# MacPhobos/audio-ident

Hardware: AMD Instinct MI355X
Metric: audio-seconds fingerprinted/sec/GPU; landmark-hash bit-exact vs CPU ref (higher is better)
Workload: dtype f32; 1 GPU; BASELINE configs[1]: 256 x 10 s 44.1 kHz mono clips, fingerprint extraction per GPU; clips_per_gpu=256, n_fft=2048, hop=512, parallelism=clip-sharded x1 (no data-path collective)

## Files before the change

audio-ident_amd/csrc/aidfp_extract.h:

```cpp
#pragma once
#include "aidfp_buffers.h"
#include "aidfp_extract_plan.h"

namespace aid {

struct Extractor {
    DevBuf<float> pcm_stage, power;
    DevBuf<uint64_t> mask, hotw;
    DevBuf<uint32_t> clip_qmax;
    DevBuf<uint32_t> k2_cold;
    HostBuf<uint64_t> h_cold;
    uint64_t *h_cold_dev = nullptr;
    DevBuf<int64_t> chunk_counts, counts;
    DevBuf<uint64_t> records;
    DevBuf<ClipDesc> desc;
    HostBuf<ClipDesc> h_desc;
    size_t desc_n = 0;
    ClipDesc *desc_dev = nullptr;
    Event desc_ev, stage_ev;
    hipStream_t stage_stream = nullptr;
    K2Policy k2;
    int64_t k2_slots[2] = {1, 1};
    int64_t k1_slots = 1;
    int64_t plane_rows = 0;
    ExtractPlan plan;
    bool have_result = false;
};

}
```

audio-ident_amd/csrc/aidfp_launch.h:

```cpp
#pragma once
#include <hip/hip_runtime.h>
#include <stdint.h>

#include "aidfp_device.h"

namespace aid {
void launch_stft_power(const void *pcm, bool s16, const ClipDesc *clips, int n_clips, int64_t f0, int64_t total_frames,
                       int64_t total_strips, int64_t slots, int hop, const Tables *tab, float *out, bool logmag,
                       uint64_t *hot, float thr, bool keep_power, uint32_t *qmax, hipStream_t s);
int peak_pick_blocks_per_cu(int width);
void launch_peak_pick(int width, const float *power, const ClipDesc *clips, int n_clips, int64_t f0, int64_t total_strips,
                      int strip_len, float thr, const uint64_t *hot, uint64_t *mask, uint32_t *cold_cnt,
                      const uint32_t *clip_qmax, float rel, hipStream_t s);
void launch_landmarks(const uint64_t *mask, const ClipDesc *clips, int n_clips, int64_t total_chunks,
                      int64_t *chunk_counts, uint64_t *records, int64_t *clip_counts, bool write, uint32_t *k2_cold,
                      uint64_t *k2_cold_host, uint32_t k2_waves, uint32_t k2_strips, bool one_chunk_each,
                      hipStream_t s);
void launch_synth(float *out, const uint32_t *tracks, const int64_t *starts, int n_clips, int64_t n, int sr,
                  int noise_a, uint32_t salt, int fmax_hz, bool envelope, const int16_t *sin_tab, hipStream_t s);
void launch_resample(const void *src, bool s16, int64_t in_base, int64_t n, int channels, int up, int down, int hl,
                     int J, const float *taps, float *dst, int64_t m_first, int64_t count, hipStream_t s,
                     int n_streams = 1, int64_t src_stride = 0, int64_t dst_stride = 0, const void *hist = nullptr,
                     int64_t hist_n = 0, int64_t hist_stride = 0);
struct SpeedVarDev;
void launch_resample_speeds(const void *src, bool s16, int channels, const int64_t *clip_off, const SpeedVarDev *vars,
                            int n_speeds, const int64_t *blk_first, const int64_t *dst_off, int pair0, int n_pairs,
                            int64_t blocks, int64_t lds_floats, float *dst, hipStream_t s);
void launch_s16_to_f32(const int16_t *src, int64_t n, float *dst, hipStream_t s);
int dedup_chunks(int64_t n_cat);
void launch_dedup_scan(const uint32_t *cw, const int64_t *coff, const double *cdur, int64_t n_cat, const uint32_t *qw,
                       const int64_t *qoff, const double *qlo, const double *qhi, int nq, double *part_sim,
                       int64_t *part_idx, double *best_sim, int64_t *best_idx, hipStream_t s);
void launch_dedup_pairs(const uint32_t *aw, const int64_t *aoff, const uint32_t *bw, const int64_t *boff, int n,
                        double *sim, hipStream_t s);
void launch_index_count(const uint32_t *ph, const uint32_t *ptrack, int64_t n, const uint8_t *tomb, uint32_t n_tracks,
                        uint32_t *cnt, hipStream_t s);
void launch_index_scatter(const uint32_t *ph, const uint32_t *ptrack, const uint32_t *pt, int64_t n,
                          const uint8_t *tomb, uint32_t n_tracks, uint32_t *cursor, uint64_t *post, hipStream_t s);
void launch_scan(const uint32_t *in, uint32_t *out, int64_t n, uint32_t *tmp, hipStream_t s);
int match_lds_blocks_per_cu();
size_t radix_scratch_u32(int64_t n);
hipError_t launch_index_sort_build(const uint32_t *ph, const uint32_t *ptrack, const uint32_t *pt, int64_t n,
                                   const uint8_t *tomb, uint32_t n_tracks, uint32_t *keys0, uint32_t *keys1,
                                   uint64_t *vals0, uint64_t *vals1, uint32_t *scratch, uint32_t *E, uint32_t *offsets,
                                   unsigned long long *nz, uint64_t **vals_out, uint16_t *sig, int rank_mode,
                                   hipStream_t s);
void launch_make_sig(const uint64_t *post, int64_t n, uint16_t *sig, hipStream_t s);
// ... 48 lines not shown
```

audio-ident_amd/csrc/aidfp_layout.h:

```cpp
#pragma once
#include <stdint.h>

namespace aid {

constexpr int kN = 2048;
constexpr int kBins = 1024;
constexpr int kPeakDT = 7;
constexpr int kPeakDF = 15;
constexpr int kZoneDT = 63;
constexpr int kZoneDF = 127;
constexpr int kFan = 10;
constexpr int kMaskWords = kBins / 64;

constexpr int kStftWaves = 16;
constexpr int kStftStrip = 16;
constexpr int kK1MinFrames = 2;
constexpr int kStftLdsPerWave = 1092;

constexpr int kPeakStripMin = 16;
constexpr int kPeakStripMax = 65536;

inline int peak_strip_len(const int64_t *frames, int n, int64_t slots) {
    int64_t fmax = 0;
    for (int c = 0; c < n; ++c) fmax = frames[c] > fmax ? frames[c] : fmax;
    auto count = [&](int64_t L) {
        int64_t k = 0;
        for (int c = 0; c < n; ++c) k += (frames[c] + L - 1) / L;
        return k;
    };
    int64_t lo = kPeakStripMin, hi = fmax > lo ? fmax : lo;
    if (hi > kPeakStripMax) hi = kPeakStripMax;
    if (count(lo) <= slots) return (int)lo;
    while (lo < hi) {
        const int64_t mid = (lo + hi) / 2;
        if (count(mid) <= slots) hi = mid; else lo = mid + 1;
    }
    return (int)lo;
}

constexpr int hot_bit(int c) { return c < 32 ? c : 95 - c; }

__host__ __device__ constexpr uint32_t bucket_key(uint32_t h) {
    return (((h >> 22) & 0xFFu) << 18) | ((h >> 30) << 16) | (((h >> 12) & 0x7Fu) << 9) | (((h >> 19) & 0x7u) << 6) |
           (h & 0x3Fu);
}

__host__ __device__ constexpr uint16_t posting_sig(uint32_t track, uint32_t t) {
    return (uint16_t)(((track * 0x9E3779B1u) >> 16) + t);
}

constexpr int64_t kLdsMaxVotes = (int64_t)1 << 18;

constexpr int kHashChunk = 1024;
constexpr int kHashChunkPeakCap = 64 * ((kHashChunk + kZoneDT + 7) / 8);

inline int64_t num_frames(int64_t n, int hop) { return (hop <= 0 || n < kN) ? 0 : 1 + (n - kN) / hop; }
inline int64_t peak_capacity(int64_t F) { return 64 * ((F + 7) / 8); }
inline int64_t hash_capacity(int64_t F) { return kFan * peak_capacity(F); }

struct ClipDesc {
    int64_t pcm_off;
    int64_t frames;
    int64_t frame_base;
    int64_t strip_base;
    int64_t chunk_base;
    int64_t hash_base;
    int64_t hash_cap;
    int64_t stft_base;
};

}
```

audio-ident_amd/csrc/extract.cpp:

```cpp
#include <cstring>

#include "engine_internal.h"

int extract_locked(aid_engine *e, const void *pcm, PcmFmt fmt, const int64_t *offsets, int32_t n_clips, int32_t loc,
                   void *stream, const int64_t *ends) {
    if (ends && loc != AID_PCM_DEVICE) return fail(AID_ERR_INVALID, "extract: clip ends need device PCM");
    HIP_TRY(hipSetDevice(e->device));
    Extractor &x = e->ext;
    ExtractPlan &p = x.plan;
    hipStream_t s = pick_stream(e, stream);
    const bool keep_power = (e->cfg.flags & AID_FLAG_KEEP_POWER) != 0, rel = e->cfg.peak_rel > 0.0f;
    if (e->last_stream && e->last_stream != s) HIP_TRY(hipStreamSynchronize(e->last_stream));
    x.have_result = false;
    const uint64_t cw = x.h_cold.p ? *reinterpret_cast<volatile uint64_t *>(x.h_cold.p) : 0;
    const uint64_t sw = x.h_cold.p ? *reinterpret_cast<volatile uint64_t *>(x.h_cold.p + 1) : 0;
    const K2Choice k2 = x.k2.choose(cw, sw);
    plan_extract(p, offsets, ends, n_clips, loc, e->cfg.hop, x.plane_rows, keep_power,
                 x.k2_slots[k2.width == 2 ? 0 : 1], k2.slots_x, k2.width);
    int64_t plane = 1;
    for (const ClipGroup &g : p.groups) plane = std::max(plane, g.frames);
    HIP_TRY(x.desc.reserve((size_t)n_clips + 1));
    HIP_TRY(x.power.reserve((size_t)plane * kBins));
    HIP_TRY(x.mask.reserve((size_t)p.total_frames * kMaskWords));
    HIP_TRY(x.hotw.reserve((size_t)p.total_frames + 1));
    if (rel) {
        HIP_TRY(x.clip_qmax.reserve((size_t)n_clips + 1));
        if (n_clips > 0) HIP_TRY(hipMemsetAsync(x.clip_qmax.p, 0, sizeof(uint32_t) * (size_t)n_clips, s));
    }
    if (!x.h_cold.p) {
        HIP_TRY(x.k2_cold.reserve(128));
        HIP_TRY(hipMemsetAsync(x.k2_cold.p, 0, 128 * sizeof(uint32_t), s));
        HIP_TRY(x.h_cold.reserve(2, hipHostMallocMapped));
        x.h_cold.p[0] = x.h_cold.p[1] = 0;
        HIP_TRY(hipHostGetDevicePointer((void **)&x.h_cold_dev, x.h_cold.p, 0));
    }
    HIP_TRY(x.chunk_counts.reserve((size_t)p.chunks + 1));
    HIP_TRY(x.records.reserve((size_t)p.records + 1));
    HIP_TRY(x.counts.reserve((size_t)n_clips + 1));
    const void *dpcm = pcm;
    if (p.staged > 0) {
        if (x.stage_stream != s) HIP_TRY(x.stage_ev.wait());
        x.stage_ev.live = false;
        const size_t nbytes = (size_t)p.staged * pcm_size(fmt);
        HIP_TRY(x.pcm_stage.reserve((nbytes + sizeof(float) - 1) / sizeof(float)));
        HIP_TRY(hipMemcpyAsync(x.pcm_stage.p, pcm_at(pcm, fmt, offsets[0]), nbytes, hipMemcpyHostToDevice, s));
        dpcm = x.pcm_stage.p;
    }
    if (n_clips > 0 && (x.desc_dev != x.desc.p || desc_differ(p.desc.data(), (size_t)n_clips, x.h_desc.p, x.desc_n))) {
        x.desc_dev = nullptr;
        HIP_TRY(x.desc_ev.wait());
        HIP_TRY(x.h_desc.reserve((size_t)n_clips + 1));
        std::memcpy(x.h_desc.p, p.desc.data(), sizeof(ClipDesc) * n_clips);
        HIP_TRY(hipMemcpyAsync(x.desc.p, x.h_desc.p, sizeof(ClipDesc) * n_clips, hipMemcpyHostToDevice, s));
        HIP_TRY(x.desc_ev.record(s));
        x.desc_n = (size_t)n_clips;
        x.desc_dev = x.desc.p;
    }
    if (p.empty_clip || p.total_frames == 0)
        HIP_TRY(hipMemsetAsync(x.counts.p, 0, sizeof(int64_t) * ((size_t)n_clips + 1), s));
    if (p.total_frames > 0) {
        for (const ClipGroup &g : p.groups) {
            if (g.frames == 0) continue;
            uint32_t *qmax = rel ? x.clip_qmax.p + g.first : nullptr;
            {
                ProfScope ps(e, AID_K_STFT, s, true);
                launch_stft_power(dpcm, fmt == kS16, x.desc.p + g.first, g.n, g.frame0, g.frames, g.k1_strips,
                                  x.k1_slots, e->cfg.hop, e->d_tab.p, x.power.p, false, x.hotw.p,
                                  e->cfg.peak_threshold, keep_power, qmax, s);
            }
            if (loc == AID_PCM_HOST && &g == &p.groups.back()) {
                HIP_TRY(x.stage_ev.record(s));
                x.stage_stream = s;
            }
            {
                ProfScope ps(e, AID_K_PEAKS, s, true);
                launch_peak_pick(p.width, x.power.p, x.desc.p + g.first, g.n, g.frame0, g.strips, g.strip_len,
                                 e->cfg.peak_threshold, x.hotw.p, x.mask.p, x.k2_cold.p, qmax, e->cfg.peak_rel, s);
            }
        }
        if (p.multi_chunk) {
            ProfScope ps(e, AID_K_LANDMARK_COUNT, s, true);
            launch_landmarks(x.mask.p, x.desc.p, n_clips, p.chunks, x.chunk_counts.p, x.records.p, x.counts.p, false,
                             nullptr, nullptr, 0u, 0u, p.one_chunk_each, s);
        }
        {
            ProfScope ps(e, AID_K_LANDMARK_WRITE, s, true);
            launch_landmarks(x.mask.p, x.desc.p, n_clips, p.chunks, x.chunk_counts.p, x.records.p, x.counts.p, true,
                             x.h_cold_dev ? x.k2_cold.p : nullptr, x.h_cold_dev, (uint32_t)(p.width * p.strips),
                             (uint32_t)p.strips, p.one_chunk_each, s);
        }
    }
    HIP_TRY(hipGetLastError());
    e->last_stream = s;
    x.have_result = true;
    return AID_OK;
}

static int result_ready(aid_engine *e, const int32_t *clip, bool wait = true) {
    if (!e) return fail(AID_ERR_INVALID, "null engine");
    if (!e->ext.have_result) return fail(AID_ERR_STATE, "no extraction yet");
    if (clip && (*clip < 0 || *clip >= e->ext.plan.n_clips)) return fail(AID_ERR_INVALID, "clip index out of range");
    return wait ? aid_sync(e) : AID_OK;
}

template <typename T>
static int read_rows(aid_engine *e, int32_t clip, const T *plane, int per, T *out, int64_t cap) {
    const ClipDesc &d = e->ext.plan.desc[clip];
    if (d.frames * per > cap) return fail(AID_ERR_INVALID, "output capacity too small");
    if (d.frames > 0)
        HIP_TRY(hipMemcpy(out, plane + d.frame_base * per, d.frames * per * sizeof(T), hipMemcpyDeviceToHost));
    return AID_OK;
}

extern "C" {

int64_t aid_num_frames(const aid_engine *e, int64_t n) { return e ? num_frames(n, e->cfg.hop) : 0; }
int64_t aid_hash_capacity(const aid_engine *e, int64_t n) { return e ? hash_capacity(num_frames(n, e->cfg.hop)) : 0; }

static int extract_entry(const char *fn, aid_engine *e, const void *pcm, PcmFmt fmt, const int64_t *offsets,
                         int32_t n_clips, int32_t loc, void *stream) {
// ... 46 lines not shown
    if (counts_dev) *counts_dev = e->ext.counts.p;
    if (clip_base_host) *clip_base_host = e->ext.plan.hash_base.data();
    if (n_clips) *n_clips = e->ext.plan.n_clips;
    return AID_OK;
}

int aid_result_power(aid_engine *e, int32_t clip, float *out, int64_t cap) {
    if (int rc = result_ready(e, &clip)) return rc;
    if (!(e->cfg.flags & AID_FLAG_KEEP_POWER))
        return fail(AID_ERR_STATE, "aid_result_power: engine created without AID_FLAG_KEEP_POWER (cold blocks not stored)");
    if (int rc = read_rows(e, clip, e->ext.power.p, kBins, out, cap)) return rc;
    for (int64_t i = 0; i < e->ext.plan.frames[clip] * kBins; ++i) out[i] = out[i] * 0.25f;
    return AID_OK;
}

int aid_result_thresholds(aid_engine *e, float *out) {
    if (int rc = result_ready(e, nullptr)) return rc;
    const int n = e->ext.plan.n_clips;
    if (n > 0 && !out) return fail(AID_ERR_INVALID, "null argument");
    const float thr = e->cfg.peak_threshold, r = e->cfg.peak_rel;
    std::vector<uint32_t> q((size_t)n, 0u);
    if (r > 0.0f && n > 0) HIP_TRY(hipMemcpy(q.data(), e->ext.clip_qmax.p, sizeof(uint32_t) * n, hipMemcpyDeviceToHost));
    for (int c = 0; c < n; ++c) {
        float qm;
        std::memcpy(&qm, &q[c], sizeof(qm));
        const float t = r * (qm * 0.25f);
        out[c] = t > thr ? t : thr;
    }
    return AID_OK;
}

int aid_result_peakmask(aid_engine *e, int32_t clip, uint64_t *out, int64_t cap) {
    if (int rc = result_ready(e, &clip)) return rc;
    return read_rows(e, clip, e->ext.mask.p, kMaskWords, out, cap);
}

int aid_spectrogram(aid_engine *e, const float *pcm, int64_t n, float *out, int64_t cap) {
    if (!e || (n > 0 && !pcm) || n < 0) return fail(AID_ERR_INVALID, "aid_spectrogram: bad argument");
    const int64_t F = num_frames(n, e->cfg.hop);
    if (F * kBins > cap) return fail(AID_ERR_INVALID, "output capacity too small");
    if (F == 0) return AID_OK;
    EngineCall call(e, nullptr, false, kDrainLast);
    if (call.rc) return call.rc;
    hipStream_t s = call.s;
    DevBuf<float> d_pcm, d_out;
    DevBuf<ClipDesc> d_desc;
    ClipDesc d{};
    d.frames = F;
    HIP_TRY(d_pcm.reserve((size_t)n));
    hipError_t he = d_out.reserve((size_t)(F * kBins));
    if (he == hipSuccess) he = d_desc.reserve(1);
    if (he == hipSuccess) he = hipMemcpy(d_pcm.p, pcm, n * sizeof(float), hipMemcpyHostToDevice);
    if (he == hipSuccess) he = hipMemcpy(d_desc.p, &d, sizeof(ClipDesc), hipMemcpyHostToDevice);
    if (he == hipSuccess)
        launch_stft_power(d_pcm.p, false, d_desc.p, 1, 0, F, (F + kStftStrip - 1) / kStftStrip, e->ext.k1_slots,
                          e->cfg.hop, e->d_tab.p, d_out.p, true, nullptr, e->cfg.peak_threshold, true, nullptr, s);
    if (he == hipSuccess) he = hipGetLastError();
    if (he == hipSuccess) he = hipStreamSynchronize(s);
    if (he == hipSuccess) he = hipMemcpy(out, d_out.p, F * kBins * sizeof(float), hipMemcpyDeviceToHost);
    return he == hipSuccess ? AID_OK : fail(AID_ERR_DEVICE, std::string("aid_spectrogram: ") + hipGetErrorString(he));
}

}
```

audio-ident_amd/csrc/landmarks.hip:

```cpp
#include "aidfp_device.h"
#include "aidfp_launch.h"

namespace aid {

constexpr int kK3 = 512;

__device__ __forceinline__ int64_t block_excl_scan(int64_t v, int64_t *tmp , int64_t *total) {
    const int tid = threadIdx.x, lane = tid & 63, w = tid >> 6;
    int64_t x = v;
#pragma unroll
    for (int off = 1; off < 64; off <<= 1) {
        const int64_t y = __shfl_up(x, off, 64);
        if (lane >= off) x += y;
    }
    if (lane == 63) tmp[w] = x;
    __syncthreads();
    int64_t base = 0, tot = 0;
#pragma unroll
    for (int i = 0; i < kK3 / 64; ++i) {
        const int64_t t = tmp[i];
        base += i < w ? t : 0;
        tot += t;
    }
    if (total) *total = tot;
    __syncthreads();
    return base + x - v;
}

__device__ __forceinline__ uint32_t make_hash(int k1, int k2, int dt) {
    return ((uint32_t)(k1 & 0x3FF) << 22) | ((uint32_t)(k2 & 0x3FF) << 12) | ((uint32_t)dt & 0xFFF);
}

template <bool WRITE>
__global__ __launch_bounds__(kK3) void k_landmarks(const uint64_t *__restrict__ mask, const ClipDesc *__restrict__ clips,
                                                  int n_clips, int64_t total_chunks, int64_t *__restrict__ chunk_counts,
                                                  uint64_t *__restrict__ records, int64_t *__restrict__ clip_counts,
                                                  uint32_t *__restrict__ k2_cold, uint64_t *__restrict__ k2_cold_host,
                                                  uint32_t k2_waves, uint32_t k2_strips, int one_chunk_each) {
    __shared__ uint32_t plist[kHashChunkPeakCap];
    __shared__ uint32_t foff[kHashChunk + kZoneDT + 2];
    __shared__ int64_t scan_tmp[kK3];
    const int tid = threadIdx.x;
    const int64_t chunk = blockIdx.x;
    if (WRITE && k2_cold && blockIdx.x == 0 && tid < 64) {
        uint32_t c = k2_cold[tid], c2 = k2_cold[64 + tid];
        k2_cold[tid] = 0u;
        k2_cold[64 + tid] = 0u;
        for (int o = 32; o > 0; o >>= 1) {
            c += __shfl_xor(c, o);
            c2 += __shfl_xor(c2, o);
        }
        if (tid == 0) {
            volatile uint64_t *h = reinterpret_cast<volatile uint64_t *>(k2_cold_host);
            h[0] = (uint64_t)c | ((uint64_t)k2_waves << 32);
            h[1] = (uint64_t)c2 | ((uint64_t)k2_strips << 32);
        }
    }
    if (chunk >= total_chunks) return;
    int lo = 0, hi = n_clips - 1;
    if (one_chunk_each) lo = (int)chunk;
    while (lo < hi) {
        const int mid = (lo + hi + 1) >> 1;
        if (clips[mid].chunk_base <= chunk) lo = mid; else hi = mid - 1;
    }
    const ClipDesc cd = clips[lo];
    const int64_t F = cd.frames;
    const int64_t q = chunk - cd.chunk_base;
    const int64_t c0 = q * kHashChunk;
    const int64_t c1 = min(c0 + (int64_t)kHashChunk, F);
    const int64_t g1 = min(c1 + (int64_t)kZoneDT, F);
    const int nf = (int)(g1 - c0);
    const uint64_t *Mc = mask + (cd.frame_base + c0) * kMaskWords;
    const int64_t nck = (F + kHashChunk - 1) / kHashChunk;
    if (!WRITE && nck == 1) return;

    const int per = (nf + kK3 - 1) / kK3;
    const int fa = min(tid * per, nf), fz = min(fa + per, nf);
    int64_t mine = 0;
    for (int f = fa; f < fz; ++f) {
        uint32_t c = 0;
#pragma unroll
        for (int w = 0; w < kMaskWords; ++w) c += __popcll(Mc[f * kMaskWords + w]);
        foff[f] = c;
        mine += c;
    }
    int64_t npk = 0;
    int64_t run = block_excl_scan(mine, scan_tmp, &npk);
    for (int f = fa; f < fz; ++f) {
        const uint32_t c = foff[f];
        foff[f] = (uint32_t)run;
        if (c == 0) continue;
        int64_t idx = run;
        uint64_t W[kMaskWords];
#pragma unroll
        for (int w = 0; w < kMaskWords; ++w) W[w] = Mc[f * kMaskWords + w];
#pragma unroll
        for (int b = 0; b < 4; ++b) {
            const uint64_t w1 = W[4 * b + 1], w2 = W[4 * b + 2], w3 = W[4 * b + 3];
            for (uint64_t m = W[4 * b] | w1 | w2 | w3; m; m &= m - 1) {
                const int l = __ffsll((unsigned long long)m) - 1;
                const int i = (int)((w1 >> l) & 1) + 2 * (int)((w2 >> l) & 1) + 3 * (int)((w3 >> l) & 1);
                plist[idx++] = ((uint32_t)f << 10) | (uint32_t)(256 * b + 4 * l + i);
            }
        }
        run += c;
    }
    if (tid == 0) foff[nf] = (uint32_t)npk;
    __syncthreads();
    const int n_anchor = (int)foff[c1 - c0];

    const int pa_per = (n_anchor + kK3 - 1) / kK3;
    const int aa = min(tid * pa_per, n_anchor), az = min(aa + pa_per, n_anchor);
    int64_t my = 0;
    uint64_t tmask = 0;
    bool tmask_ok = false;
    for (int i = aa; i < az; ++i) {
        const uint32_t a = plist[i];
        const int ta = (int)(a >> 10), ka = (int)(a & 1023);
        int got = 0;
        uint64_t mk = 0;
        bool ok = true;
        for (int j = i + 1; j < (int)npk && got < kFan; ++j) {
            const uint32_t b = plist[j];
            const int dt = (int)(b >> 10) - ta;
            if (dt > kZoneDT) break;
            if (dt <= 0) continue;
            const int df = (int)(b & 1023) - ka;
            if (df < -kZoneDF || df > kZoneDF) continue;
            if (j - i - 1 < 64) mk |= 1ull << (j - i - 1);
            else ok = false;
            ++got;
        }
        if (i == aa) {
            tmask = mk;
            tmask_ok = ok;
        }
        my += got;
    }
    int64_t chunk_total = 0;
    const int64_t excl = block_excl_scan(my, scan_tmp, &chunk_total);
    if constexpr (!WRITE) {
        if (tid == 0) chunk_counts[chunk] = chunk_total;
// ... 12 lines not shown
                block_excl_scan(all, scan_tmp, &tot);
                if (tid == 0) clip_counts[lo] = tot;
            }
        }
        uint64_t *out = records + cd.hash_base + before + excl;
        int64_t o = 0;
        for (int i = aa; i < az; ++i) {
            const uint32_t a = plist[i];
            const int ta = (int)(a >> 10), ka = (int)(a & 1023);
            const uint64_t t1 = (uint64_t)(c0 + ta) << 32;
            if (i == aa && tmask_ok) {
                for (uint64_t m = tmask; m; m &= m - 1) {
                    const uint32_t b = plist[i + 1 + (__ffsll((unsigned long long)m) - 1)];
                    out[o++] = t1 | make_hash(ka, (int)(b & 1023), (int)(b >> 10) - ta);
                }
                continue;
            }
            int got = 0;
            for (int j = i + 1; j < (int)npk && got < kFan; ++j) {
                const uint32_t b = plist[j];
                const int dt = (int)(b >> 10) - ta;
                if (dt > kZoneDT) break;
                if (dt <= 0) continue;
                const int kb = (int)(b & 1023);
                const int df = kb - ka;
                if (df < -kZoneDF || df > kZoneDF) continue;
                out[o++] = t1 | make_hash(ka, kb, dt);
                ++got;
            }
        }
    }
}

void launch_landmarks(const uint64_t *mask, const ClipDesc *clips, int n_clips, int64_t total_chunks,
                      int64_t *chunk_counts, uint64_t *records, int64_t *clip_counts, bool write, uint32_t *k2_cold,
                      uint64_t *k2_cold_host, uint32_t k2_waves, uint32_t k2_strips, bool one_chunk_each,
                      hipStream_t s) {
    if (total_chunks <= 0) return;
    if (write)
        timed_launch(k_landmarks<true>, dim3((unsigned)total_chunks), dim3(kK3), 0, s, mask, clips, n_clips,
                           total_chunks, chunk_counts, records, clip_counts, k2_cold, k2_cold_host, k2_waves,
                     k2_strips, one_chunk_each ? 1 : 0);
    else
        timed_launch(k_landmarks<false>, dim3((unsigned)total_chunks), dim3(kK3), 0, s, mask, clips, n_clips,
                           total_chunks, chunk_counts, records, clip_counts, (uint32_t *)nullptr, (uint64_t *)nullptr, 0u,
                     0u, one_chunk_each ? 1 : 0);
}

}
```

audio-ident_amd/csrc/peaks.hip:

```cpp
#include "aidfp_device.h"
#include "aidfp_launch.h"

namespace aid {

constexpr int kRowsPerStep = 4;

#if defined(AID_K2_STAMPS)
__device__ unsigned long long g_k2_stamps[8];
#define AID_K2_T() ((unsigned long long)__builtin_amdgcn_s_memtime())
#endif

template <int LANE>
__device__ __forceinline__ uint32_t write_lane(uint32_t v, uint32_t s_val) {
    asm volatile("v_writelane_b32 %0, %1, %2" : "+v"(v) : "s"(s_val), "i"(LANE));
    return v;
}

__device__ __forceinline__ int pkey(float x) {
    float r;
    asm("v_max_f32 %0, 0, %1" : "=v"(r) : "v"(x));
    return __float_as_int(r);
}

struct PeakPickArgs {
    const float *power;
    const ClipDesc *clips;
    int n_clips;
    int64_t f0, total_strips;
    int strip_len;
    float thr;
    const uint64_t *hot;
    uint64_t *mask;
    uint32_t *cold_cnt;
    const uint32_t *clip_qmax;
    float rel;
};

template <int W>
#if defined(AID_K2_PF2) && defined(AID_K2_OCC3)
__global__ __launch_bounds__(64 * W, 3) void k_peak_pick(
#else
__global__ __launch_bounds__(64 * W, 4) void k_peak_pick(
#endif
                                                  const float *__restrict__ power_, const ClipDesc *__restrict__ clips_,
                                                  int n_clips_, int64_t f0_, int64_t total_strips_, int strip_len_, float thr_,
                                                  const uint64_t *__restrict__ hot_, uint64_t *__restrict__ mask_,
                                                  uint32_t *__restrict__ cold_cnt_,
                                                  const uint32_t *__restrict__ clip_qmax_, float rel_) {
    static_assert(W == 2 || W == 4, "quarter waves per workgroup");
    constexpr int kGB = 256 * W;
    __shared__ __attribute__((aligned(16))) int rows[kRowsPerStep][kGB + 32];
    __shared__ __attribute__((aligned(16))) int bms[kRowsPerStep][64 * W + 8];
#pragma unroll
    for (int g = 0; g < 4 / W; ++g) {
        const float *power = power_;
        const ClipDesc *clips = clips_;
        int n_clips = n_clips_, strip_len = strip_len_;
        int64_t f0 = f0_, total_strips = total_strips_;
        float thr = thr_, rel = rel_;
        const uint64_t *hot = hot_;
        uint64_t *mask = mask_;
        uint32_t *cold_cnt = cold_cnt_;
        const uint32_t *clip_qmax = clip_qmax_;
        if (g > 0) {
            typedef const __attribute__((address_space(4))) PeakPickArgs *ArgPtr;
            ArgPtr a = (ArgPtr)__builtin_amdgcn_kernarg_segment_ptr();
            asm volatile("" : "+s"(a));
            power = a->power, clips = a->clips, n_clips = a->n_clips, f0 = a->f0, total_strips = a->total_strips;
            strip_len = a->strip_len, thr = a->thr, hot = a->hot, mask = a->mask, cold_cnt = a->cold_cnt;
            clip_qmax = a->clip_qmax, rel = a->rel;
            __syncthreads();
        }
#if defined(AID_K2_STAMPS)
        const unsigned long long st_birth = AID_K2_T();
        unsigned long long st_bar = 0, st_b0 = 0, st_b1 = 0;
#endif
        const int lane = threadIdx.x & 63;
        const int wl = __builtin_amdgcn_readfirstlane(((int)(threadIdx.x >> 6) + (int)blockIdx.x) & (W - 1));
        const int wave = wl + W * g;
        const int tid = wave * 64 + lane;
        const int lt = wl * 64 + lane;
        constexpr int kInf = 0x7F800000;

        int64_t strip;
        {
            const int64_t nb = gridDim.x, b = blockIdx.x;
            const int64_t per = nb / 8, rem = nb % 8, x = b % 8, y = b / 8;
            strip = (x < rem ? x * (per + 1) : rem * (per + 1) + (x - rem) * per) + y;
            strip = nb - 1 - strip;
        }
        if (strip >= total_strips) return;
        int lo = 0, hi = n_clips - 1;
        while (lo < hi) {
            const int mid = (lo + hi + 1) >> 1;
            if (clips[mid].strip_base <= strip) lo = mid; else hi = mid - 1;
        }
        const int F = (int)clips[lo].frames;
        const int64_t fb = clips[lo].frame_base;
        const int t0 = (int)(strip - clips[lo].strip_base) * strip_len;
        const int t1 = min(t0 + strip_len, F);
        const float *P = power + (fb - f0) * kBins;
        uint64_t *M = mask + fb * kMaskWords + 4 * wave + lane;
        int kthr = __float_as_int(4.0f * thr);
        if (clip_qmax) kthr = max(kthr, __float_as_int(rel * __uint_as_float(clip_qmax[lo])));

        const int rbeg = t0 - kPeakDT;
        const int iters = (t1 - t0) + 2 * kPeakDT;
        const uint64_t *HW = hot + fb;
        auto hotword = [&](int r) -> uint64_t { return (r >= 0 && r < F) ? HW[r] : 0ull; };
        auto hotwords = [&](int rb) -> uint64_t {
            const int r = rb + (lane & 3);
            return (r >= 0 && r < F) ? HW[r] : 0ull;
        };
        auto word_of = [](uint64_t v, int j) -> uint64_t {
            return ((uint64_t)(uint32_t)__builtin_amdgcn_readlane((int)(v >> 32), j) << 32) |
                   (uint32_t)__builtin_amdgcn_readlane((int)v, j);
        };

        const int bwl = g == 0 ? W - 1 : 0;

        if constexpr (W == 4) {
            if (tid < 16) {
#pragma unroll
                for (int r = 0; r < kRowsPerStep; ++r) {
                    rows[r][tid] = 0;
                    rows[r][kBins + 16 + tid] = 0;
                    if (tid < 4) {
                        bms[r][tid] = 0;
                        bms[r][260 + tid] = 0;
                    }
                }
            }
        } else if (lane < 16) {
#pragma unroll
            for (int r = 0; r < kRowsPerStep; ++r) {
// ... 4 lines not shown
                if (wl == W - 1) {
                    rows[r][kGB + 16 + lane] = 0;
                    if (lane < 4) bms[r][64 * W + 4 + lane] = 0;
                }
            }
        }

        int m2r[8][4];
        int pend[8][4];
        int fprev[4], m7p[4];
#pragma unroll
        for (int s = 0; s < 8; ++s)
#pragma unroll
            for (int i = 0; i < 4; ++i) { m2r[s][i] = 0; pend[s][i] = -1; }
#pragma unroll
        for (int i = 0; i < 4; ++i) { fprev[i] = 0; m7p[i] = 0; }
        const uint64_t b0ok = __ballot(tid != 0);

        const int myb = hot_bit(tid >> 2);
        uint64_t wmask = 0;
        for (int c = max(16 * wave - 1, 0); c <= min(16 * wave + 16, 63); ++c) wmask |= 1ull << hot_bit(c);
        bool need2 = false, bhot = false;
        {
            uint64_t acc = 0;
            for (int r = rbeg + lane; r < rbeg + iters; r += 64) acc |= (r >= 0 && r < F) ? HW[r] : 0ull;
            bool cold = __ballot((acc & wmask) != 0ull) == 0;
            if (W < 4) {
                bhot = __ballot((acc >> hot_bit(g == 0 ? 16 * W : 16 * W - 1)) & 1ull) != 0;
                if (g == 0) {
                    uint64_t up = 0;
                    for (int c = 16 * W - 1; c < 64; ++c) up |= 1ull << hot_bit(c);
                    need2 = __ballot((acc & up) != 0ull) != 0;
                    if (!need2) {
                        uint64_t *Mz = mask + fb * kMaskWords + 4 * (W + wl) + (lane & 3);
                        for (int r = t0 + (lane >> 2); r < t1; r += 16) Mz[(int64_t)r * kMaskWords] = 0;
                    } else {
                        cold = false;
                        if (wl == 0 && lane == 0 && cold_cnt) atomicAdd(&cold_cnt[64 + (blockIdx.x & 63)], 1u);
                    }
                }
            }
            if (cold) {
#pragma unroll
                for (int j = 0; j < kRowsPerStep; ++j) {
                    reinterpret_cast<int4 *>(&rows[j][16])[lt] = make_int4(0, 0, 0, 0);
                    bms[j][4 + lt] = 0;
                }
                uint64_t *Mz = mask + fb * kMaskWords + 4 * wave + (lane & 3);
                for (int r = t0 + (lane >> 2); r < t1; r += 16) Mz[(int64_t)r * kMaskWords] = 0;
                if (lane == 0 && cold_cnt && g == 0) atomicAdd(&cold_cnt[blockIdx.x & 63], 1u);
#if defined(AID_K2_STAMPS)
                if (lane == 0) atomicAdd(&g_k2_stamps[7], 1ull);
#endif
                asm volatile("s_waitcnt lgkmcnt(0)" ::: "memory");
                return;
            }
        }
        const int rlo = max(rbeg, 0), rhi = min(rbeg + iters, F);
        constexpr uint32_t kOOB = 0x80000000u;
        const __amdgpu_buffer_rsrc_t rows_rsrc = __builtin_amdgcn_make_buffer_rsrc(
            const_cast<float *>(P + (int64_t)rlo * kBins), (short)0, (rhi - rlo) * kBins * 4, 0x00020000);
        auto load_row = [&](int r, uint64_t hwr) -> float4 {
            const uint32_t off = ((hwr >> myb) & 1ull) ? (uint32_t)(r - rlo) * (kBins * 4) + 16u * tid : kOOB;
            const auto v = __builtin_amdgcn_raw_buffer_load_b128(rows_rsrc, off, 0, 0);
            return make_float4(__int_as_float(v[0]), __int_as_float(v[1]), __int_as_float(v[2]), __int_as_float(v[3]));
        };
#if defined(AID_K2_PF2)
        float4 pfb[2][kRowsPerStep];
        uint64_t hs[2][kRowsPerStep], hcur[kRowsPerStep];
#pragma unroll
        for (int b = 0; b < 2; ++b)
#pragma unroll
            for (int j = 0; j < kRowsPerStep; ++j) {
                const int r = rbeg + b * kRowsPerStep + j;
                hs[b][j] = hotword(r);
                pfb[b][j] = load_row(r, b * kRowsPerStep + j < iters ? hs[b][j] : 0ull);
                hcur[j] = 0ull;
            }
        uint64_t hwv = hotwords(rbeg + 2 * kRowsPerStep);
#else
        float4 pf[kRowsPerStep];
#pragma unroll
// ... 93 lines not shown
                const int mpre1 = max(me.x, me.y), mpre2 = max(mpre1, me.z);
                const int msuf2 = max(me.z, me.w), msuf1 = max(me.y, msuf2);
                int L[4], R[4];
                L[0] = max(lsuf1, M3L);
                L[1] = max(max(lsuf2, M3L), me.x);
                L[2] = max(max(lf.w, M3L), mpre1);
                L[3] = max(M3L, mpre2);
                R[0] = max(msuf1, M3R);
                R[1] = max(max(msuf2, M3R), rt.x);
                R[2] = max(max(me.w, M3R), rpre1);
                R[3] = max(M3R, rpre2);
                const int mev[4] = {me.x, me.y, me.z, me.w};

                const int thr_row = (r >= t0 && r < t1) ? kthr : kInf;
#pragma unroll
                for (int i = 0; i < 4; ++i) {
                    const int p = mev[i];
                    const int fm = max(max(L[i], p), R[i]);
                    const int m2 = max(fm, fprev[i]);
                    fprev[i] = fm;
                    const int bf = max(max(L[i], thr_row), m7p[i]);
                    m2r[s][i] = m2;
                    const int m7 = max(max(max(m2, m2r[(s - 2) & 7][i]), m2r[(s - 4) & 7][i]), m2r[(s - 5) & 7][i]);
                    m7p[i] = m7;
                    pk[i] = pend[(s + 1) & 7][i] >= m7;
                    bal[i] = __ballot(pk[i]);
                    bool cand = p > bf && p >= R[i];
                    if (i == 0) cand = cand && ((b0ok >> lane) & 1ull);
                    pend[s][i] = cand ? p : -1;
                }
                }
                const uint64_t b0 = bal[0], b1 = bal[1], b2 = bal[2], b3 = bal[3];
                const int rd = r - kPeakDT;
                if (rd >= t0 && rd < t1) {
                    uint32_t lo, hi;
                    asm volatile("" : "=v"(lo), "=v"(hi));
                    lo = write_lane<0>(lo, (uint32_t)b0);
                    hi = write_lane<0>(hi, (uint32_t)(b0 >> 32));
                    lo = write_lane<1>(lo, (uint32_t)b1);
                    hi = write_lane<1>(hi, (uint32_t)(b1 >> 32));
                    lo = write_lane<2>(lo, (uint32_t)b2);
                    hi = write_lane<2>(hi, (uint32_t)(b2 >> 32));
                    lo = write_lane<3>(lo, (uint32_t)b3);
                    hi = write_lane<3>(hi, (uint32_t)(b3 >> 32));
                    if (lane < 4) M[(int64_t)rd * kMaskWords] = ((uint64_t)hi << 32) | lo;
                }
            }
        }
#if defined(AID_K2_STAMPS)
        {
            const unsigned long long t = AID_K2_T();
            st_bar += st_b1 - st_b0;
            if (lane == 0) {
                atomicAdd(&g_k2_stamps[0], st_bar);
                atomicAdd(&g_k2_stamps[5], 1ull);
                atomicAdd(&g_k2_stamps[6], t - st_birth);
            }
        }
#endif
        if (!need2) break;
    }
}

#if defined(AID_K2_STAMPS)
int k2_stamps_read(unsigned long long *out, bool reset) {
    if (hipMemcpyFromSymbol(out, HIP_SYMBOL(g_k2_stamps), sizeof(unsigned long long) * 8) != hipSuccess) return -2;
    if (reset) {
        const unsigned long long z[8] = {};
        if (hipMemcpyToSymbol(HIP_SYMBOL(g_k2_stamps), z, sizeof(z)) != hipSuccess) return -2;
    }
    return 0;
}
#endif

void launch_peak_pick(int width, const float *power, const ClipDesc *clips, int n_clips, int64_t f0, int64_t total_strips,
                      int strip_len, float thr, const uint64_t *hot, uint64_t *mask, uint32_t *cold_cnt,
                      const uint32_t *clip_qmax, float rel, hipStream_t s) {
    if (total_strips <= 0) return;
    if (width == 2)
        timed_launch(k_peak_pick<2>, dim3((unsigned)total_strips), dim3(128), 0, s, power, clips, n_clips, f0,
                     total_strips, strip_len, thr, hot, mask, cold_cnt, clip_qmax, rel);
    else
        timed_launch(k_peak_pick<4>, dim3((unsigned)total_strips), dim3(256), 0, s, power, clips, n_clips, f0,
                     total_strips, strip_len, thr, hot, mask, cold_cnt, clip_qmax, rel);
}

int peak_pick_blocks_per_cu(int width) {
    int n = 0;
    const hipError_t rc = width == 2 ? hipOccupancyMaxActiveBlocksPerMultiprocessor(&n, k_peak_pick<2>, 128, 0)
                                     : hipOccupancyMaxActiveBlocksPerMultiprocessor(&n, k_peak_pick<4>, 256, 0);
    if (rc != hipSuccess || n <= 0) n = 1;
    return n;
}

}
```

Measured before the change: 6.762 million audio-s/s.

## Replace dense peak bitmask with compact per-strip peak lists

```diff
diff --git a/audio-ident_amd/csrc/aidfp_extract.h b/audio-ident_amd/csrc/aidfp_extract.h
--- a/audio-ident_amd/csrc/aidfp_extract.h
+++ b/audio-ident_amd/csrc/aidfp_extract.h
@@ -1,12 +1,20 @@
 #pragma once
 #include "aidfp_buffers.h"
 #include "aidfp_extract_plan.h"
+#include "aidfp_peaklist.h"
 
 namespace aid {
 
 struct Extractor {
     DevBuf<float> pcm_stage, power;
-    DevBuf<uint64_t> mask, hotw;
+    DevBuf<uint64_t> hotw;
+    DevBuf<uint32_t> list_entries, list_counts;
+    DevBuf<ClipLists> clip_lists;
+    HostBuf<ClipLists> h_clip_lists;
+    size_t clip_lists_n = 0;
+    ClipLists *clip_lists_dev = nullptr;
+    Event clip_lists_ev;
+    PeakListPlan lists;
     DevBuf<uint32_t> clip_qmax;
     DevBuf<uint32_t> k2_cold;
     HostBuf<uint64_t> h_cold;
diff --git a/audio-ident_amd/csrc/aidfp_launch.h b/audio-ident_amd/csrc/aidfp_launch.h
--- a/audio-ident_amd/csrc/aidfp_launch.h
+++ b/audio-ident_amd/csrc/aidfp_launch.h
@@ -10,9 +10,10 @@
                        uint64_t *hot, float thr, bool keep_power, uint32_t *qmax, hipStream_t s);
 int peak_pick_blocks_per_cu(int width);
 void launch_peak_pick(int width, const float *power, const ClipDesc *clips, int n_clips, int64_t f0, int64_t total_strips,
-                      int strip_len, float thr, const uint64_t *hot, uint64_t *mask, uint32_t *cold_cnt,
+                      int strip_len, float thr, const uint64_t *hot, uint32_t *lists, uint32_t *counts, uint32_t *cold_cnt,
                       const uint32_t *clip_qmax, float rel, hipStream_t s);
-void launch_landmarks(const uint64_t *mask, const ClipDesc *clips, int n_clips, int64_t total_chunks,
+void launch_landmarks(const uint32_t *lists, const uint32_t *list_counts, const ClipLists *clip_lists,
+                      const ClipDesc *clips, int n_clips, int64_t total_chunks,
                       int64_t *chunk_counts, uint64_t *records, int64_t *clip_counts, bool write, uint32_t *k2_cold,
                       uint64_t *k2_cold_host, uint32_t k2_waves, uint32_t k2_strips, bool one_chunk_each,
                       hipStream_t s);
diff --git a/audio-ident_amd/csrc/aidfp_layout.h b/audio-ident_amd/csrc/aidfp_layout.h
--- a/audio-ident_amd/csrc/aidfp_layout.h
+++ b/audio-ident_amd/csrc/aidfp_layout.h
@@ -54,6 +54,15 @@
 constexpr int kHashChunk = 1024;
 constexpr int kHashChunkPeakCap = 64 * ((kHashChunk + kZoneDT + 7) / 8);
 
+constexpr int kPeakFrameBits = 22;
+constexpr int64_t peaklist_cap(int64_t strip_len) { return 16 * ((strip_len + 7) / 8); }
+struct ClipLists {
+    int64_t entry_base;
+    int32_t strip0;
+    int32_t strip_len;
+};
+constexpr int kHashChunkLists = 4 * ((kHashChunk + kZoneDT - 2) / kPeakStripMin + 2);
+
 inline int64_t num_frames(int64_t n, int hop) { return (hop <= 0 || n < kN) ? 0 : 1 + (n - kN) / hop; }
 inline int64_t peak_capacity(int64_t F) { return 64 * ((F + 7) / 8); }
 inline int64_t hash_capacity(int64_t F) { return kFan * peak_capacity(F); }
diff --git a/audio-ident_amd/csrc/aidfp_peaklist.h b/audio-ident_amd/csrc/aidfp_peaklist.h
--- /dev/null
+++ b/audio-ident_amd/csrc/aidfp_peaklist.h
@@ -0,0 +1,59 @@
+#pragma once
+#include <string.h>
+
+#include <vector>
+
+#include "aidfp_extract_plan.h"
+#include "aidfp_layout.h"
+
+namespace aid {
+
+struct GroupLists {
+    int64_t strip0 = 0, entry0 = 0;
+};
+
+struct PeakListPlan {
+    std::vector<ClipLists> clips;
+    std::vector<GroupLists> groups;
+    int64_t strips = 0;
+    int64_t entries = 0;
+};
+
+inline void plan_peaklists(PeakListPlan &l, const ExtractPlan &p) {
+    l.clips.resize(p.n_clips);
+    l.groups.resize(p.groups.size());
+    l.strips = l.entries = 0;
+    for (size_t gi = 0; gi < p.groups.size(); ++gi) {
+        const ClipGroup &g = p.groups[gi];
+        const int64_t cap = peaklist_cap(g.strip_len);
+        l.groups[gi] = {l.strips, l.entries};
+        for (int c = g.first; c < g.first + g.n; ++c)
+            l.clips[c] = {l.entries + 4 * p.desc[c].strip_base * cap, (int32_t)(l.strips + p.desc[c].strip_base),
+                          (int32_t)g.strip_len};
+        l.strips += g.strips;
+        l.entries += 4 * g.strips * cap;
+    }
+}
+
+inline bool lists_differ(const ClipLists *a, size_t na, const ClipLists *b, size_t nb) {
+    return na != nb || (na > 0 && memcmp(a, b, na * sizeof(ClipLists)) != 0);
+}
+
+inline int64_t clip_strips(int64_t frames, int64_t strip_len) { return (frames + strip_len - 1) / strip_len; }
+
+inline void peaklists_to_mask(const uint32_t *counts, const uint32_t *entries, int64_t n_strips, int64_t cap,
+                              int64_t frames, uint64_t *out) {
+    for (int64_t i = 0; i < frames * kMaskWords; ++i) out[i] = 0;
+    for (int64_t li = 0; li < 4 * n_strips; ++li) {
+        const int64_t n = counts[li] < cap ? counts[li] : cap;
+        for (int64_t j = 0; j < n; ++j) {
+            const uint32_t e = entries[li * cap + j];
+            const int64_t f = e >> 10;
+            const int bin = (int)(e & 1023u);
+            if (f >= frames) continue;
+            out[f * kMaskWords + 4 * (bin >> 8) + (bin & 3)] |= 1ull << ((bin & 255) >> 2);
+        }
+    }
+}
+
+}
diff --git a/audio-ident_amd/csrc/extract.cpp b/audio-ident_amd/csrc/extract.cpp
--- a/audio-ident_amd/csrc/extract.cpp
+++ b/audio-ident_amd/csrc/extract.cpp
@@ -17,11 +17,18 @@
     const K2Choice k2 = x.k2.choose(cw, sw);
     plan_extract(p, offsets, ends, n_clips, loc, e->cfg.hop, x.plane_rows, keep_power,
                  x.k2_slots[k2.width == 2 ? 0 : 1], k2.slots_x, k2.width);
+    for (int c = 0; c < n_clips; ++c)
+        if (p.frames[c] >= ((int64_t)1 << kPeakFrameBits))
+            return fail(AID_ERR_INVALID, "extract: a clip of 2^22 frames or more");
+    PeakListPlan &pl = x.lists;
+    plan_peaklists(pl, p);
     int64_t plane = 1;
     for (const ClipGroup &g : p.groups) plane = std::max(plane, g.frames);
     HIP_TRY(x.desc.reserve((size_t)n_clips + 1));
     HIP_TRY(x.power.reserve((size_t)plane * kBins));
-    HIP_TRY(x.mask.reserve((size_t)p.total_frames * kMaskWords));
+    HIP_TRY(x.list_entries.reserve((size_t)pl.entries + 1));
+    HIP_TRY(x.list_counts.reserve((size_t)pl.strips * 4 + 1));
+    HIP_TRY(x.clip_lists.reserve((size_t)n_clips + 1));
     HIP_TRY(x.hotw.reserve((size_t)p.total_frames + 1));
     if (rel) {
         HIP_TRY(x.clip_qmax.reserve((size_t)n_clips + 1));
@@ -56,11 +63,23 @@
         x.desc_n = (size_t)n_clips;
         x.desc_dev = x.desc.p;
     }
+    if (n_clips > 0 && (x.clip_lists_dev != x.clip_lists.p ||
+                        lists_differ(pl.clips.data(), (size_t)n_clips, x.h_clip_lists.p, x.clip_lists_n))) {
+        x.clip_lists_dev = nullptr;
+        HIP_TRY(x.clip_lists_ev.wait());
+        HIP_TRY(x.h_clip_lists.reserve((size_t)n_clips + 1));
+        std::memcpy(x.h_clip_lists.p, pl.clips.data(), sizeof(ClipLists) * n_clips);
+        HIP_TRY(hipMemcpyAsync(x.clip_lists.p, x.h_clip_lists.p, sizeof(ClipLists) * n_clips, hipMemcpyHostToDevice, s));
+        HIP_TRY(x.clip_lists_ev.record(s));
+        x.clip_lists_n = (size_t)n_clips;
+        x.clip_lists_dev = x.clip_lists.p;
+    }
     if (p.empty_clip || p.total_frames == 0)
         HIP_TRY(hipMemsetAsync(x.counts.p, 0, sizeof(int64_t) * ((size_t)n_clips + 1), s));
     if (p.total_frames > 0) {
         for (const ClipGroup &g : p.groups) {
             if (g.frames == 0) continue;
+            const GroupLists &gl = pl.groups[&g - p.groups.data()];
             uint32_t *qmax = rel ? x.clip_qmax.p + g.first : nullptr;
             {
                 ProfScope ps(e, AID_K_STFT, s, true);
@@ -75,17 +94,18 @@
             {
                 ProfScope ps(e, AID_K_PEAKS, s, true);
                 launch_peak_pick(p.width, x.power.p, x.desc.p + g.first, g.n, g.frame0, g.strips, g.strip_len,
-                                 e->cfg.peak_threshold, x.hotw.p, x.mask.p, x.k2_cold.p, qmax, e->cfg.peak_rel, s);
+                                 e->cfg.peak_threshold, x.hotw.p, x.list_entries.p + gl.entry0, x.list_counts.p + 4 * gl.strip0,
+                                 x.k2_cold.p, qmax, e->cfg.peak_rel, s);
             }
         }
         if (p.multi_chunk) {
             ProfScope ps(e, AID_K_LANDMARK_COUNT, s, true);
-            launch_landmarks(x.mask.p, x.desc.p, n_clips, p.chunks, x.chunk_counts.p, x.records.p, x.counts.p, false,
+            launch_landmarks(x.list_entries.p, x.list_counts.p, x.clip_lists.p, x.desc.p, n_clips, p.chunks, x.chunk_counts.p, x.records.p, x.counts.p, false,
                              nullptr, nullptr, 0u, 0u, p.one_chunk_each, s);
         }
         {
             ProfScope ps(e, AID_K_LANDMARK_WRITE, s, true);
-            launch_landmarks(x.mask.p, x.desc.p, n_clips, p.chunks, x.chunk_counts.p, x.records.p, x.counts.p, true,
+            launch_landmarks(x.list_entries.p, x.list_counts.p, x.clip_lists.p, x.desc.p, n_clips, p.chunks, x.chunk_counts.p, x.records.p, x.counts.p, true,
                              x.h_cold_dev ? x.k2_cold.p : nullptr, x.h_cold_dev, (uint32_t)(p.width * p.strips),
                              (uint32_t)p.strips, p.one_chunk_each, s);
         }
@@ -198,7 +218,19 @@
 
 int aid_result_peakmask(aid_engine *e, int32_t clip, uint64_t *out, int64_t cap) {
     if (int rc = result_ready(e, &clip)) return rc;
-    return read_rows(e, clip, e->ext.mask.p, kMaskWords, out, cap);
+    const Extractor &x = e->ext;
+    const int64_t F = x.plan.frames[clip];
+    if (F * kMaskWords > cap) return fail(AID_ERR_INVALID, "output capacity too small");
+    if (F == 0) return AID_OK;
+    const ClipLists &cl = x.lists.clips[clip];
+    const int64_t ns = clip_strips(F, cl.strip_len), lcap = peaklist_cap(cl.strip_len);
+    std::vector<uint32_t> counts((size_t)(4 * ns)), entries((size_t)(4 * ns * lcap));
+    HIP_TRY(hipMemcpy(counts.data(), x.list_counts.p + 4 * (int64_t)cl.strip0, counts.size() * sizeof(uint32_t),
+                      hipMemcpyDeviceToHost));
+    HIP_TRY(hipMemcpy(entries.data(), x.list_entries.p + cl.entry_base, entries.size() * sizeof(uint32_t),
+                      hipMemcpyDeviceToHost));
+    peaklists_to_mask(counts.data(), entries.data(), ns, lcap, F, out);
+    return AID_OK;
 }
 
 int aid_spectrogram(aid_engine *e, const float *pcm, int64_t n, float *out, int64_t cap) {
diff --git a/audio-ident_amd/csrc/landmarks.hip b/audio-ident_amd/csrc/landmarks.hip
--- a/audio-ident_amd/csrc/landmarks.hip
+++ b/audio-ident_amd/csrc/landmarks.hip
@@ -31,15 +31,31 @@
     return ((uint32_t)(k1 & 0x3FF) << 22) | ((uint32_t)(k2 & 0x3FF) << 12) | ((uint32_t)dt & 0xFFF);
 }
 
+template <typename P>
+__device__ __forceinline__ int lower_bound(P a, int n, uint32_t key) {
+    int lo = 0, hi = n;
+    while (lo < hi) {
+        const int mid = (lo + hi) >> 1;
+        if (a[mid] < key) lo = mid + 1; else hi = mid;
+    }
+    return lo;
+}
+
 template <bool WRITE>
-__global__ __launch_bounds__(kK3) void k_landmarks(const uint64_t *__restrict__ mask, const ClipDesc *__restrict__ clips,
+__global__ __launch_bounds__(kK3) void k_landmarks(const uint32_t *__restrict__ lists,
+                                                  const uint32_t *__restrict__ list_counts,
+                                                  const ClipLists *__restrict__ clip_lists,
+                                                  const ClipDesc *__restrict__ clips,
                                                   int n_clips, int64_t total_chunks, int64_t *__restrict__ chunk_counts,
                                                   uint64_t *__restrict__ records, int64_t *__restrict__ clip_counts,
                                                   uint32_t *__restrict__ k2_cold, uint64_t *__restrict__ k2_cold_host,
                                                   uint32_t k2_waves, uint32_t k2_strips, int one_chunk_each) {
+    static_assert(kHashChunkLists <= kK3, "one thread per list of a chunk");
     __shared__ uint32_t plist[kHashChunkPeakCap];
-    __shared__ uint32_t foff[kHashChunk + kZoneDT + 2];
-    __shared__ int64_t scan_tmp[kK3];
+    __shared__ uint16_t lfrm[kHashChunkPeakCap];
+    __shared__ uint16_t loff[kHashChunkLists + 2];
+    __shared__ uint32_t lskip[4];
+    __shared__ int64_t scan_tmp[kK3 / 64];
     const int tid = threadIdx.x;
     const int64_t chunk = blockIdx.x;
     if (WRITE && k2_cold && blockIdx.x == 0 && tid < 64) {
@@ -69,45 +85,65 @@
     const int64_t c0 = q * kHashChunk;
     const int64_t c1 = min(c0 + (int64_t)kHashChunk, F);
     const int64_t g1 = min(c1 + (int64_t)kZoneDT, F);
-    const int nf = (int)(g1 - c0);
-    const uint64_t *Mc = mask + (cd.frame_base + c0) * kMaskWords;
     const int64_t nck = (F + kHashChunk - 1) / kHashChunk;
     if (!WRITE && nck == 1) return;
 
-    const int per = (nf + kK3 - 1) / kK3;
-    const int fa = min(tid * per, nf), fz = min(fa + per, nf);
+    const ClipLists cl = clip_lists[lo];
+    const int L = cl.strip_len, cap = (int)peaklist_cap(L);
+    const int sa = (int)(c0 / L), ns = (int)((g1 - 1) / L) - sa + 1;
+    const uint32_t klo = (uint32_t)c0 << 10, khi = (uint32_t)g1 << 10;
     int64_t mine = 0;
-    for (int f = fa; f < fz; ++f) {
-        uint32_t c = 0;
+    int skip = 0;
+    if (tid < 4 * ns) {
+        const int s = sa + (tid >> 2);
+        const uint32_t *mylist = lists + cl.entry_base + ((int64_t)4 * s + (tid & 3)) * cap;
+        int n = min((int)list_counts[4 * ((int64_t)cl.strip0 + s) + (tid & 3)], cap);
+        if (min((int64_t)(s + 1) * L, F) > g1) n = lower_bound(mylist, n, khi);
+        if ((int64_t)s * L < c0) skip = lower_bound(mylist, n, klo);
+        mine = n - skip;
+        if (tid < 4) lskip[tid] = (uint32_t)skip;
+    }
+    int64_t npk = 0;
+    const int64_t run = min(block_excl_scan(mine, scan_tmp, &npk), (int64_t)kHashChunkPeakCap);
+    npk = min(npk, (int64_t)kHashChunkPeakCap);
+    if (tid < 4 * ns) loff[tid] = (uint16_t)run;
+    if (tid == 4 * ns) loff[tid] = (uint16_t)npk;
+    __syncthreads();
+    auto list_of = [&](int x) {
+        int a = 0, b = 4 * ns - 1;
+        while (a < b) {
+            const int mid = (a + b + 1) >> 1;
+            if ((int)loff[mid] <= x) a = mid; else b = mid - 1;
+        }
+        return a;
+    };
+    auto entry = [&](int x, int l) {
+        return lists[cl.entry_base + ((int64_t)4 * (sa + (l >> 2)) + (l & 3)) * cap + (l < 4 ? lskip[l] : 0u) +
+                     (x - (int)loff[l])];
+    };
+    int l_first = 0;
+    uint32_t key_first = 0;
+    for (int x = tid; x < (int)npk; x += kK3) {
+        const int l = list_of(x);
+        const uint32_t key = entry(x, l);
+        if (x == tid) l_first = l, key_first = key;
+        lfrm[x] = (uint16_t)((key - klo) >> 10);
+    }
+    __syncthreads();
+    for (int x = tid; x < (int)npk; x += kK3) {
+        const int l = x == tid ? l_first : list_of(x), l0 = l & ~3;
+        const uint32_t key = x == tid ? key_first : entry(x, l);
+        const uint32_t f = (uint16_t)((key - klo) >> 10);
+        int rank = (int)loff[l0] + (x - (int)loff[l]);
 #pragma unroll
-        for (int w = 0; w < kMaskWords; ++w) c += __popcll(Mc[f * kMaskWords + w]);
-        foff[f] = c;
-        mine += c;
-    }
-    int64_t npk = 0;
-    int64_t run = block_excl_scan(mine, scan_tmp, &npk);
-    for (int f = fa; f < fz; ++f) {
-        const uint32_t c = foff[f];
-        foff[f] = (uint32_t)run;
-        if (c == 0) continue;
-        int64_t idx = run;
-        uint64_t W[kMaskWords];
-#pragma unroll
-        for (int w = 0; w < kMaskWords; ++w) W[w] = Mc[f * kMaskWords + w];
-#pragma unroll
-        for (int b = 0; b < 4; ++b) {
-            const uint64_t w1 = W[4 * b + 1], w2 = W[4 * b + 2], w3 = W[4 * b + 3];
-            for (uint64_t m = W[4 * b] | w1 | w2 | w3; m; m &= m - 1) {
-                const int l = __ffsll((unsigned long long)m) - 1;
-                const int i = (int)((w1 >> l) & 1) + 2 * (int)((w2 >> l) & 1) + 3 * (int)((w3 >> l) & 1);
-                plist[idx++] = ((uint32_t)f << 10) | (uint32_t)(256 * b + 4 * l + i);
-            }
-        }
-        run += c;
-    }
-    if (tid == 0) foff[nf] = (uint32_t)npk;
-    __syncthreads();
-    const int n_anchor = (int)foff[c1 - c0];
+        for (int w = 0; w < 4; ++w) {
+            const int o = (int)loff[l0 + w], n = (int)loff[l0 + w + 1] - o;
+            if (l0 + w != l && n > 0) rank += lower_bound(lfrm + o, n, f + (l0 + w < l ? 1u : 0u));
+        }
+        plist[min(rank, kHashChunkPeakCap - 1)] = key - klo;
+    }
+    __syncthreads();
+    const int n_anchor = g1 > c1 ? lower_bound(plist, (int)npk, (uint32_t)(c1 - c0) << 10) : (int)npk;
 
     const int pa_per = (n_anchor + kK3 - 1) / kK3;
     const int aa = min(tid * pa_per, n_anchor), az = min(aa + pa_per, n_anchor);
@@ -186,17 +222,18 @@
     }
 }
 
-void launch_landmarks(const uint64_t *mask, const ClipDesc *clips, int n_clips, int64_t total_chunks,
+void launch_landmarks(const uint32_t *lists, const uint32_t *list_counts, const ClipLists *clip_lists,
+                      const ClipDesc *clips, int n_clips, int64_t total_chunks,
                       int64_t *chunk_counts, uint64_t *records, int64_t *clip_counts, bool write, uint32_t *k2_cold,
                       uint64_t *k2_cold_host, uint32_t k2_waves, uint32_t k2_strips, bool one_chunk_each,
                       hipStream_t s) {
     if (total_chunks <= 0) return;
     if (write)
-        timed_launch(k_landmarks<true>, dim3((unsigned)total_chunks), dim3(kK3), 0, s, mask, clips, n_clips,
+        timed_launch(k_landmarks<true>, dim3((unsigned)total_chunks), dim3(kK3), 0, s, lists, list_counts, clip_lists, clips, n_clips,
                            total_chunks, chunk_counts, records, clip_counts, k2_cold, k2_cold_host, k2_waves,
                      k2_strips, one_chunk_each ? 1 : 0);
     else
-        timed_launch(k_landmarks<false>, dim3((unsigned)total_chunks), dim3(kK3), 0, s, mask, clips, n_clips,
+        timed_launch(k_landmarks<false>, dim3((unsigned)total_chunks), dim3(kK3), 0, s, lists, list_counts, clip_lists, clips, n_clips,
                            total_chunks, chunk_counts, records, clip_counts, (uint32_t *)nullptr, (uint64_t *)nullptr, 0u,
                      0u, one_chunk_each ? 1 : 0);
 }
diff --git a/audio-ident_amd/csrc/peaks.hip b/audio-ident_amd/csrc/peaks.hip
--- a/audio-ident_amd/csrc/peaks.hip
+++ b/audio-ident_amd/csrc/peaks.hip
@@ -9,12 +9,6 @@
 __device__ unsigned long long g_k2_stamps[8];
 #define AID_K2_T() ((unsigned long long)__builtin_amdgcn_s_memtime())
 #endif
-
-template <int LANE>
-__device__ __forceinline__ uint32_t write_lane(uint32_t v, uint32_t s_val) {
-    asm volatile("v_writelane_b32 %0, %1, %2" : "+v"(v) : "s"(s_val), "i"(LANE));
-    return v;
-}
 
 __device__ __forceinline__ int pkey(float x) {
     float r;
@@ -30,7 +24,7 @@
     int strip_len;
     float thr;
     const uint64_t *hot;
-    uint64_t *mask;
+    uint32_t *lists, *counts;
     uint32_t *cold_cnt;
     const uint32_t *clip_qmax;
     float rel;
@@ -44,8 +38,8 @@
 #endif
                                                   const float *__restrict__ power_, const ClipDesc *__restrict__ clips_,
                                                   int n_clips_, int64_t f0_, int64_t total_strips_, int strip_len_, float thr_,
-                                                  const uint64_t *__restrict__ hot_, uint64_t *__restrict__ mask_,
-                                                  uint32_t *__restrict__ cold_cnt_,
+                                                  const uint64_t *__restrict__ hot_, uint32_t *__restrict__ lists_,
+                                                  uint32_t *__restrict__ counts_, uint32_t *__restrict__ cold_cnt_,
                                                   const uint32_t *__restrict__ clip_qmax_, float rel_) {
     static_assert(W == 2 || W == 4, "quarter waves per workgroup");
     constexpr int kGB = 256 * W;
@@ -59,7 +53,7 @@
         int64_t f0 = f0_, total_strips = total_strips_;
         float thr = thr_, rel = rel_;
         const uint64_t *hot = hot_;
-        uint64_t *mask = mask_;
+        uint32_t *lists = lists_, *counts = counts_;
         uint32_t *cold_cnt = cold_cnt_;
         const uint32_t *clip_qmax = clip_qmax_;
         if (g > 0) {
@@ -67,8 +61,8 @@
             ArgPtr a = (ArgPtr)__builtin_amdgcn_kernarg_segment_ptr();
             asm volatile("" : "+s"(a));
             power = a->power, clips = a->clips, n_clips = a->n_clips, f0 = a->f0, total_strips = a->total_strips;
-            strip_len = a->strip_len, thr = a->thr, hot = a->hot, mask = a->mask, cold_cnt = a->cold_cnt;
-            clip_qmax = a->clip_qmax, rel = a->rel;
+            strip_len = a->strip_len, thr = a->thr, hot = a->hot, lists = a->lists, counts = a->counts;
+            cold_cnt = a->cold_cnt, clip_qmax = a->clip_qmax, rel = a->rel;
             __syncthreads();
         }
 #if defined(AID_K2_STAMPS)
@@ -100,7 +94,10 @@
         const int t0 = (int)(strip - clips[lo].strip_base) * strip_len;
         const int t1 = min(t0 + strip_len, F);
         const float *P = power + (fb - f0) * kBins;
-        uint64_t *M = mask + fb * kMaskWords + 4 * wave + lane;
+        const int lcap = 16 * ((strip_len + 7) >> 3);
+        uint32_t *LP = lists + (strip * 4 + wave) * lcap;
+        uint32_t *const CP = counts + strip * 4;
+        int npk = 0;
         int kthr = __float_as_int(4.0f * thr);
         if (clip_qmax) kthr = max(kthr, __float_as_int(rel * __uint_as_float(clip_qmax[lo])));
 
@@ -171,8 +168,7 @@
                     for (int c = 16 * W - 1; c < 64; ++c) up |= 1ull << hot_bit(c);
                     need2 = __ballot((acc & up) != 0ull) != 0;
                     if (!need2) {
-                        uint64_t *Mz = mask + fb * kMaskWords + 4 * (W + wl) + (lane & 3);
-                        for (int r = t0 + (lane >> 2); r < t1; r += 16) Mz[(int64_t)r * kMaskWords] = 0;
+                        if (lane == 0) CP[W + wl] = 0u;
                     } else {
                         cold = false;
                         if (wl == 0 && lane == 0 && cold_cnt) atomicAdd(&cold_cnt[64 + (blockIdx.x & 63)], 1u);
@@ -185,8 +181,7 @@
                     reinterpret_cast<int4 *>(&rows[j][16])[lt] = make_int4(0, 0, 0, 0);
                     bms[j][4 + lt] = 0;
                 }
-                uint64_t *Mz = mask + fb * kMaskWords + 4 * wave + (lane & 3);
-                for (int r = t0 + (lane >> 2); r < t1; r += 16) Mz[(int64_t)r * kMaskWords] = 0;
+                if (lane == 0) CP[wave] = 0u;
                 if (lane == 0 && cold_cnt && g == 0) atomicAdd(&cold_cnt[blockIdx.x & 63], 1u);
 #if defined(AID_K2_STAMPS)
                 if (lane == 0) atomicAdd(&g_k2_stamps[7], 1ull);
@@ -346,18 +341,16 @@
                 }
                 const uint64_t b0 = bal[0], b1 = bal[1], b2 = bal[2], b3 = bal[3];
                 const int rd = r - kPeakDT;
-                if (rd >= t0 && rd < t1) {
-                    uint32_t lo, hi;
-                    asm volatile("" : "=v"(lo), "=v"(hi));
-                    lo = write_lane<0>(lo, (uint32_t)b0);
-                    hi = write_lane<0>(hi, (uint32_t)(b0 >> 32));
-                    lo = write_lane<1>(lo, (uint32_t)b1);
-                    hi = write_lane<1>(hi, (uint32_t)(b1 >> 32));
-                    lo = write_lane<2>(lo, (uint32_t)b2);
-                    hi = write_lane<2>(hi, (uint32_t)(b2 >> 32));
-                    lo = write_lane<3>(lo, (uint32_t)b3);
-                    hi = write_lane<3>(hi, (uint32_t)(b3 >> 32));
-                    if (lane < 4) M[(int64_t)rd * kMaskWords] = ((uint64_t)hi << 32) | lo;
+                const uint64_t any = b0 | b1 | b2 | b3;
+                if (any != 0ull && rd >= t0 && rd < t1) {
+                    int i, slot = npk + (int)__builtin_amdgcn_mbcnt_hi((uint32_t)(any >> 32),
+                                                                       __builtin_amdgcn_mbcnt_lo((uint32_t)any, 0u));
+                    asm("v_cndmask_b32_e64 %0, 0, 3, %1" : "=v"(i) : "s"(b3));
+                    asm("v_cndmask_b32_e64 %0, %0, 2, %1" : "+v"(i) : "s"(b2));
+                    asm("v_cndmask_b32_e64 %0, %0, 1, %1" : "+v"(i) : "s"(b1));
+                    asm("v_cndmask_b32_e64 %0, -1, %0, %1" : "+v"(slot) : "s"(any));
+                    if ((uint32_t)slot < (uint32_t)lcap) LP[slot] = ((uint32_t)rd << 10) | (uint32_t)(4 * tid + i);
+                    npk += __popcll(any);
                 }
             }
         }
@@ -372,6 +365,7 @@
             }
         }
 #endif
+        if (lane == 0) CP[wave] = (uint32_t)npk;
         if (!need2) break;
     }
 }
@@ -388,15 +382,15 @@
 #endif
 
 void launch_peak_pick(int width, const float *power, const ClipDesc *clips, int n_clips, int64_t f0, int64_t total_strips,
-                      int strip_len, float thr, const uint64_t *hot, uint64_t *mask, uint32_t *cold_cnt,
+                      int strip_len, float thr, const uint64_t *hot, uint32_t *lists, uint32_t *counts, uint32_t *cold_cnt,
                       const uint32_t *clip_qmax, float rel, hipStream_t s) {
     if (total_strips <= 0) return;
     if (width == 2)
         timed_launch(k_peak_pick<2>, dim3((unsigned)total_strips), dim3(128), 0, s, power, clips, n_clips, f0,
-                     total_strips, strip_len, thr, hot, mask, cold_cnt, clip_qmax, rel);
+                     total_strips, strip_len, thr, hot, lists, counts, cold_cnt, clip_qmax, rel);
     else
         timed_launch(k_peak_pick<4>, dim3((unsigned)total_strips), dim3(256), 0, s, power, clips, n_clips, f0,
-                     total_strips, strip_len, thr, hot, mask, cold_cnt, clip_qmax, rel);
+                     total_strips, strip_len, thr, hot, lists, counts, cold_cnt, clip_qmax, rel);
 }
 
 int peak_pick_blocks_per_cu(int width) {
```

Result: faster. 6.843 million audio-s/s (median of 5 runs) (+1.2%).
